# viswavi/speech-anonymization

Hardware: AMD Instinct MI355X
Metric: audio frames/sec (node), ConvAE+gender-adv train step (higher is better)
Workload: dtype bf16x3; 1 GPU; ConvAE recon0.1+sex0.9 adversarial train step (L1 recon + NLL), shape M: 32 utt/GPU x 161120 samples (T=1008 frames), Fbank x2 + norm + fwd + bwd + clip + Adam + Noam; batch_per_gpu=32, frames_per_utt=1008, parallelism=dp1

## Files before the change

include/sa_hip.h:

```cpp
#ifndef SA_HIP_H
#define SA_HIP_H
#ifdef __cplusplus
extern "C" {
#endif

#define SA_F32 0
#define SA_BF16 1
#define SA_BF16X3 2
#define SA_BF16X1F 3
#define SA_FP8 4
#define SA_F64 5
#define SA_MAX_TAPS 5
#define SA_COMM_ID_BYTES 128

typedef struct SaTaps {
  int ntaps[2];
  int off[2][SA_MAX_TAPS];
  int widx[2][SA_MAX_TAPS];
} SaTaps;

typedef struct SaConvArgs {
  const void* x;
  const void* wp;
  const float* bias;
// ... 19 lines not shown
} SaConvArgs;

int sa_conv_gemm(int dtype, int cin, int cout, int sa, int u, const SaConvArgs* a, void* stream);
int sa_abi_sizeof(int which);
int sa_conv_gemm_ntiles(int cin, int cout, int u, int Lout);
int sa_conv_gemm_ntiles_tm(int tile_rows, int u, int Lout);
int sa_conv_gemm_set_tile_rows(int rows);
int sa_conv_gemm_geometry(int dtype, int cin, int cout, int u, int Lout, int* ntiles, int* nslabs);
int sa_conv_gemm_set_impl(int impl);
int sa_conv_gemm_route(int dtype, int cin, int cout, int sa, int u, const SaConvArgs* a);
int sa_conv_pp_set_tile_rows(int rows);
int sa_conv_ws_set_bcost(int tiles);
int sa_conv_ws_set_xcd_weights(const unsigned char* w8);
int sa_conv_ws_calibrate_read(unsigned long long* life512x2);
int sa_conv_wsd_set_bcost(int tiles);

int sa_pack_weights(int dtype, const float* src, void* dst, int ntaps, int K, int N, int sk, int sn,
                    int st, void* stream);

typedef struct SaPackDesc {
  const float* src; void* dst;
  int dtype, ntaps, K, N, sk, sn, st, pad_;
  float* scale;
} SaPackDesc;
int sa_pack_weights_multi(const SaPackDesc* descs, int n, int blocks_per_image, void* stream);
int sa_pack_scales_multi(const SaPackDesc* descs, int n, void* stream);

typedef struct SaWgradArgs {
  const void* x;
  const void* dy;
// ... 187 lines not shown
```

speech-anonymization_amd/_lib.py:

```python
import ctypes as C
import os

import torch

_HERE = os.path.dirname(os.path.abspath(__file__))
LIB_PATH = os.environ.get("SA_HIP_LIB") or os.path.join(_HERE, "libsa_hip.so")

F32, BF16, BF16X3, BF16X1F, FP8, F64 = 0, 1, 2, 3, 4, 5
MAX_TAPS = 5

c_fp = C.POINTER(C.c_float)
vp = C.c_void_p


class SaTaps(C.Structure):
    _fields_ = [("ntaps", C.c_int * 2), ("off", (C.c_int * MAX_TAPS) * 2),
                ("widx", (C.c_int * MAX_TAPS) * 2)]


class SaConvArgs(C.Structure):
    _fields_ = [("x", vp), ("wp", vp), ("bias", vp), ("y", vp),
                ("s1", vp), ("t1", vp), ("s2", vp), ("t2", vp),
                ("swish", C.c_int), ("relu", C.c_int), ("stats", vp),
                ("B", C.c_int), ("Lin", C.c_int), ("Lout", C.c_int), ("ntiles", C.c_int),
# ... 77 lines not shown


SYMBOLS = [
    "sa_conv_gemm", "sa_abi_sizeof", "sa_conv_gemm_ntiles", "sa_conv_gemm_ntiles_tm", "sa_conv_gemm_set_tile_rows",
    "sa_conv_gemm_geometry", "sa_conv_gemm_set_impl", "sa_conv_gemm_route", "sa_conv_pp_set_tile_rows", "sa_pack_weights", "sa_pack_weights_multi", "sa_pack_scales_multi", "sa_wgrad", "sa_wgrad_kw", "sa_wgrad_reduce",
    "sa_conv1toC", "sa_conv1toC_ntiles", "sa_convCto1", "sa_wgrad1C", "sa_wgrad1C_nchunk",
    "sa_sum_slabs", "sa_ew_stats", "sa_ew_apply", "sa_ew_ntiles", "sa_act_stats",
    "sa_sum_partials", "sa_sum_rows_d", "sa_reduce_finalize", "sa_fin_in_fwd", "sa_fin_bn_fwd", "sa_fin_bn_eval", "sa_fin_norm_bwd", "sa_fin_bias",
    "sa_pool_fwd", "sa_pool_nseg", "sa_pool_gather", "sa_pool_fin", "sa_pool_bwd", "sa_dense", "sa_colsums",
    "sa_bn2d_bwd", "sa_dense_wgrad", "sa_log_softmax", "sa_log_softmax_bwd",
    "sa_loss_workspace_bytes", "sa_recon_loss", "sa_cls_losses", "sa_cosine_loss",
    "sa_tdnn_fwd", "sa_time_pool", "sa_leaky_affine", "sa_tdnn_bwd_input", "sa_tdnn_fold", "sa_time_pool_bwd",
    "sa_leaky_affine_bwd", "sa_cluster_mi", "sa_fbank", "sa_fbank_table_elems", "sa_fbank_ntiles", "sa_fbank_scratch_bytes", "sa_fbank_normalize",
    "sa_comm_unique_id", "sa_comm_init", "sa_comm_world", "sa_comm_allreduce", "sa_comm_allreduce_inline", "sa_comm_join", "sa_comm_ncalls",
    "sa_comm_destroy", "sa_head_fwd", "sa_head_bwd", "sa_head_max_rows", "sa_conv_ws_set_bcost", "sa_conv_wsd_set_bcost",
    "sa_add_layernorm_fwd", "sa_layernorm_bwd", "sa_reflect_pad_fwd", "sa_reflect_pad_bwd", "sa_ln_leaky_fwd", "sa_ln_leaky_bwd", "sa_bias_multi", "sa_asr_block0_fwd", "sa_asr_block0_bwd", "sa_conv_ws_set_xcd_weights", "sa_conv_ws_calibrate_read", "sa_wgrad_reduce_multi", "sa_clip_grads",
]

_lib = None


class SaHipError(RuntimeError):
    pass


def load():
    global _lib
    if _lib is None:
        if not os.path.exists(LIB_PATH):
            raise SaHipError(
                f"{LIB_PATH} not found: build it with `python -c 'import __graft_entry__ as g; "
# ... 52 lines not shown
```

speech-anonymization_amd/csrc/sa_conv_ws.hip:

```cpp
#include <type_traits>
#include "sa_conv_cfg.h"

#ifndef SA_ABL
#define SA_ABL 0
#endif

#ifdef SA_WS_STAMPS
__device__ unsigned long long sa_ws_dbg[64 * 8];
#define WS_STAMP(it, i) do { if (lane_ == 0 && wave_ == 0 && blockIdx.x == 7 && (it) < 64) { \
  unsigned long long t_; asm volatile("s_memtime %0\n\ts_waitcnt lgkmcnt(0)" : "=s"(t_) :: "memory"); \
  sa_ws_dbg[(it) * 8 + (i)] = t_; } } while (0)
extern "C" int sa_ws_dbg_read(unsigned long long* out) {
  return -(int)hipMemcpyFromSymbol(out, HIP_SYMBOL(sa_ws_dbg), sizeof(sa_ws_dbg));
}
#else
#define WS_STAMP(it, i)
#endif

#include "sa_conv_ws_common.h"

extern unsigned long long g_ws_xcd_weights;

namespace {

template <int MODE, int NT, int HALO, int CC = 128, int CO = CC, int SA = 1, int UU = 1>
__global__ __launch_bounds__(256) __attribute__((amdgpu_waves_per_eu(1, 1)))
void sa_conv_ws_kernel(SaConvArgs a, int bcost, int total_tiles, unsigned long long xw) {
  typedef WsGeo<CC, NT, HALO, CO, SA, UU> G;
  constexpr int WS_CO = G::CO, WS_SA = G::SA, WS_BM = G::BM;
  static_assert(UU == 1 || MODE == 0, "transposed layers: plain rows");
  constexpr int WS_C = G::C, WS_TM = G::TM, WS_KSTEPS = G::KSTEPS, WS_PITCH = G::PITCH, RPP = G::RPP, LPR = G::LPR,
                NWN = G::NWN, NWM = G::NWM;
  static_assert(CC == 128 || MODE == 0 || MODE == 1, "64 channels: plain and affine + x*sigmoid(x) prologues");
  constexpr int WS_NTAPS = G::NTAPS, WS_ROWS = G::ROWS, WS_PLANE = G::PLANE, WS_NDMA = G::NDMA, WS_DPW = G::DPW,
                WS_RAW_BYTES = G::RAW_BYTES, WS_BUF_BYTES = G::BUF_BYTES, WS_NAGPR_FRAGS = G::NAGPR_FRAGS,
                WS_FT = G::FT, WS_SUBS = G::SUBS;
  (void)WS_ROWS; (void)NWM;
  static_assert(MODE == 0 || MODE == 5 || NT == 5, "the staged transforms need the 240-slot tile");
  constexpr bool PRO2 = MODE == 2;
  constexpr bool SWISH = MODE == 1 || MODE == 3 || MODE == 4;
  constexpr bool PSTAT = MODE == 3, AFF2 = MODE == 4 || MODE == 5;
  constexpr bool COLRED = PRO2 || PSTAT;
  extern __shared__ __attribute__((aligned(16))) unsigned char smem[];
  bf16_t* const planes = reinterpret_cast<bf16_t*>(smem);
  unsigned char* const raw = smem + 2 * WS_BUF_BYTES;
  const unsigned raw_lds = (unsigned)(uintptr_t)(lds_byte*)raw;
  const int tid = threadIdx.x, lane_ = tid & 63;
  const int wave_ = __builtin_amdgcn_readfirstlane(tid >> 6);
  const int wn_ = wave_ % NWN, wm_ = wave_ / NWN;
  const int ph_ = UU == 2 ? wm_ % 2 : 0, rh_ = UU == 2 ? wm_ / 2 : wm_;
  const int ntap_ = a.taps.ntaps[ph_];
#ifdef SA_WS_OLD_RANGES
  int first, last;
  {
    const unsigned long long U = (unsigned long long)a.ntiles + 4u;
    const unsigned long long ctot = (unsigned long long)(total_tiles / a.ntiles) * U;
    auto inv = [&](unsigned long long c) {
// ... 66 lines not shown
  float bv = a.bias ? a.bias[wn_ * 32 + (lane_ & 31)] : 0.0f;
  float relu_floor = a.relu ? 0.0f : -__builtin_inff();
  const bool has_stats = a.stats != nullptr, has_ao = a.a_out != nullptr;

  const int half_ = lane_ >> 5, l31_ = lane_ & 31;
  const int rowp_ = lane_ / LPR, cq_ = lane_ % LPR;
  unsigned row0 = RPP * wave_ + rowp_;
  unsigned dma_off = wave_ * 1024 + lane_ * 16;
  unsigned raw_off = wave_ * 1024 + lane_ * 16;
  unsigned pl_off = (row0 * WS_PITCH + cq_ * 4) * 2;
  unsigned ao_off = (row0 * WS_C + cq_ * 4) * 2;
  unsigned y_off = (UU == 2 ? (8 * half_ + ph_ + 128 * rh_) * WS_CO + wn_ * 32 + l31_
                            : (4 * half_ + 64 * rh_) * WS_CO + wn_ * 32 + l31_) * 4;
  unsigned st_off = ((G::SLABS == 2 ? rh_ * WS_CO : 0) + wn_ * 32 + l31_) * 8;
  unsigned swap_off = (lane_ ^ 32) * 4;
  asm volatile("" : "+v"(bv), "+v"(relu_floor), "+v"(row0), "+v"(dma_off), "+v"(raw_off), "+v"(pl_off), "+v"(ao_off), "+v"(y_off),
               "+v"(st_off), "+v"(swap_off));

#define WS_IDS int lane = lane_, wave = wave_; asm volatile("" : "+v"(lane), "+s"(wave)); (void)wave; (void)lane

  struct Tile { int b, tile, irow, orow, srow; };
  const int slab_short = G::SLABS == 2 ? 2 * a.ntiles - (((a.Lout + UU - 1) / UU + 63) / 64) : 0;
  const int nslab_b = a.ntiles * G::SLABS - slab_short;
  auto tile_of = [&](int t) {
    Tile r; r.b = t / a.ntiles; r.tile = t - r.b * a.ntiles;
    r.irow = r.b * a.Lin + r.tile * (WS_BM * WS_SA) + a.rowmin; r.orow = r.b * a.Lout + r.tile * WS_TM;
    r.srow = r.b * nslab_b + r.tile * G::SLABS;
    return r;
  };
  const int iwrap = a.Lin - (a.ntiles - 1) * (WS_BM * WS_SA), owrap = a.Lout - (a.ntiles - 1) * WS_TM,
            swrap = nslab_b - (a.ntiles - 1) * G::SLABS;
  auto next_tile = [&](Tile T) {
// ... 173 lines not shown
      if (j == WS_DPW - 1 && wave_ + 4 * j >= WS_NDMA) return;
      if (owns(T, false, j)) {
#pragma unroll
        for (int q = 0; q < 4; ++q) { csum[q] += f[q]; csq[q] = fmaf(f[q], f[q], csq[q]); }
      }
    }
  };
  auto piece_write = [&](int j, int part = 2) {
    if (j == WS_DPW - 1 && wave_ + 4 * j >= WS_NDMA) return;
    unsigned char* dst = smem + (pl_cur + j * (4 * RPP * WS_PITCH * 2));
    if (part != 1) *reinterpret_cast<uint2*>(dst) = phi;
    if (part != 0) *reinterpret_cast<uint2*>(dst + WS_PLANE * 2) = plo;
  };
  auto piece_cache = [&](Tile T, bool edge, int j) {
    if (j == WS_DPW - 1 && wave_ + 4 * j >= WS_NDMA) return;
    if (has_ao && owns(T, edge, j)) ws_store_b64(aobase_t + j * (4 * RPP * WS_C * 2), ao_off, phi);
  };
  constexpr int NRED = PSTAT ? 2 : 1;
  auto colsum_put = [&](int it) {
    if constexpr (COLRED) {
      if (PSTAT || a.nb_colsum) {
        float* colred = reinterpret_cast<float*>(raw + (PRO2 ? 2 : 1) * WS_RAW_BYTES) + (size_t)(it & 1) * 4 * WS_C * NRED;
#pragma unroll
        for (int q = 0; q < 4; ++q) {
          const float v = csum[q] + __int_as_float(__builtin_amdgcn_ds_bpermute((int)swap_off, __float_as_int(csum[q])));
          if (lane_ < 32) colred[(wave_ * WS_C + (lane_ & 31) * 4 + q) * NRED] = v;
          csum[q] = 0.0f;
          if constexpr (PSTAT) {
            const float u = csq[q] + __int_as_float(__builtin_amdgcn_ds_bpermute((int)swap_off, __float_as_int(csq[q])));
            if (lane_ < 32) colred[(wave_ * WS_C + (lane_ & 31) * 4 + q) * NRED + 1] = u;
            csq[q] = 0.0f;
          }
        }
      }
    }
  };
  auto colsum_out = [&](int t, int it) {
    if constexpr (COLRED) {
      if ((PSTAT || a.nb_colsum) && tid < WS_C) {
        const float* colred = reinterpret_cast<const float*>(raw + (PRO2 ? 2 : 1) * WS_RAW_BYTES) + (size_t)(it & 1) * 4 * WS_C * NRED;
        float* dst = PSTAT ? a.pro_stats : a.nb_colsum;
// ... 5 lines not shown
      }
    }
  };

  f32x16 acc[2], accp[2];
  float ssum = 0.0f, ssq = 0.0f;
  auto epi_form = [&](int n) {
    float val = accp[n >> 4][n & 15] + bv;
    asm("v_max_f32 %0, %0, %1" : "+v"(val) : "v"(relu_floor));
    return val;
  };
  float eval = 0.0f;
  auto epi_store = [&](int n) {
    const int m = n >> 4, i = n & 15;
    const int ro = m * 32 + (i & 3) + 8 * (i >> 2);
    if constexpr ((SA_ABL & 64) == 0) ws_store_b32(ybase_e + ro * (UU * WS_CO * 4), y_off, eval);
  };
  auto epi_accum = [&](int n) {
    asm volatile("v_add_f32 %0, %0, %2\n\tv_fmac_f32 %1, %2, %2" : "+v"(ssum), "+v"(ssq) : "v"(eval));
    if (n + 1 < 32) eval = epi_form(n + 1);
  };
  auto epi_value = [&](Tile T, bool partial, int n) {
    if (!partial) {
      epi_store(n);
      epi_accum(n);
    } else {
      WS_IDS;
      const int m = n >> 4, i = n & 15;
      const int ro = m * 32 + (i & 3) + 8 * (i >> 2);
      const float val = epi_form(n);
      const int orow = UU == 2 ? 2 * (64 * rh_ + ro + 4 * (lane >> 5)) + ph_ : 64 * rh_ + ro + 4 * (lane >> 5);
// ... 4 lines not shown
    }
  };
  float st_s = 0.0f, st_q = 0.0f;
  bool st_slab_ok = true;
  bool st_pending = false;
  int st_it = 0;
  char* stbase_e = nullptr;
  auto epi_stats = [&](Tile T, int part = 2) {
    if (has_stats) {
      if (part != 1) {
        st_s = ssum + __int_as_float(__builtin_amdgcn_ds_bpermute((int)swap_off, __float_as_int(ssum)));
        st_q = ssq + __int_as_float(__builtin_amdgcn_ds_bpermute((int)swap_off, __float_as_int(ssq)));
      }
      if (part != 0) {
        if constexpr (G::COMBINE == 1) {
          ws_store_b64(stbase_e, st_off, make_uint2(__float_as_uint(st_s), __float_as_uint(st_q)));
        } else {
          float2* stred = reinterpret_cast<float2*>(raw + WS_RAW_BYTES) + (size_t)(st_it & 1) * 4 * 32;
          if (lane_ < 32) stred[wave_ * 32 + lane_] = make_float2(st_s, st_q);
          st_pending = true;
        }
      }
    }
    if (part != 0) { ssum = 0.0f; ssq = 0.0f; }
  };
  auto stats_out = [&]() {
    if constexpr (G::COMBINE == 2) {
      const bool leader = UU == 2 ? ph_ == 0 : wm_ == 0;
      if (st_pending && leader && st_slab_ok) {
        const float2* stred = reinterpret_cast<const float2*>(raw + WS_RAW_BYTES) + (size_t)(st_it & 1) * 4 * 32;
        const float2 p0 = stred[wave_ * 32 + (lane_ & 31)], p1 = stred[(wave_ + NWN) * 32 + (lane_ & 31)];
        ws_store_b64(stbase_e, st_off, make_uint2(__float_as_uint(p0.x + p1.x), __float_as_uint(p0.y + p1.y)));
      }
      st_pending = false;
      ++st_it;
    }
  };

  int toff[WS_NTAPS];
#pragma unroll
  for (int t = 0; t < WS_NTAPS; ++t) toff[t] = (a.taps.off[ph_][UU == 1 || t < ntap_ ? t : 0] - a.rowmin) * WS_PITCH;

  Tile Tc = tile_of(first), Tn = tile_of(first + 1 < last ? first + 1 : last - 1), Tp = Tc;
#pragma unroll
  for (int q = 0; q < 4; ++q) { csum[q] = 0.0f; csq[q] = 0.0f; }
  {
    const bool ec = is_edge(Tc), en = is_edge(Tn);
// ... 58 lines not shown
    }
    WS_STAMP(it, 0);
    auto tile_body = [&](auto fast_c) {
      constexpr bool FAST = decltype(fast_c)::value;
      auto filler = [&](auto f_c) {
        constexpr int fs = decltype(f_c)::value;
        if constexpr ((SA_ABL & 8) != 0 || !FAST) return;
        if constexpr (fs < 32) {
          epi_store(fs); epi_accum(fs);
        } else if constexpr (fs == 32 || fs == 33) {
          epi_stats(Tp, fs - 32);
        } else if constexpr (fs == 34) {
          WS_STAMP(it, 3);
        } else if constexpr (fs == WS_FT - 1) {
          WS_STAMP(it, 4);
          if (G::COMBINE == 1 && has_stats) asm volatile("s_waitcnt vmcnt(33)" ::: "memory");
          else asm volatile("s_waitcnt vmcnt(32)" ::: "memory");
          WS_STAMP(it, 5);
          piece_read(0);
        } else if constexpr (fs >= WS_FT && WS_SUBS == 18) {
          constexpr int j = (fs - WS_FT) / 18, k = (fs - WS_FT) % 18;
          constexpr int NA = AFF2 ? 7 : 6;
          if constexpr (j > 0 && (k == 6 || k == 7)) piece_write(j - 1, k - 6);
          if constexpr (k < NA) piece_level(Tn, j, k);
          if constexpr (j + 1 < WS_DPW && k == 1) piece_read(j + 1, 0);
          if constexpr (j + 1 < WS_DPW && k == 13 && PRO2) piece_read(j + 1, 1);
          if constexpr (k >= 8 && k < 12) piece_split(j, k - 8);
          if constexpr (k == 14) piece_cache(Tn, false, j);
          if constexpr (k == 15) piece_pstat(Tn, j);
          if constexpr (k == 16) dma_piece(Tnn, false, j, 0);
          if constexpr (k == 17 && PRO2) dma_piece(Tnn, false, j, 1);
        } else if constexpr (fs >= WS_FT && WS_SUBS == 4) {
          constexpr int j = (fs - WS_FT) / 4, k = (fs - WS_FT) % 4;
          if constexpr (j > 0 && k < 2) piece_write(j - 1, k);
          if constexpr (k == 0) { piece_level(Tn, j, 0); piece_split(j, 0); }
          if constexpr (j + 1 < WS_DPW && k == 1) piece_read(j + 1, 0);
          if constexpr (k == 1) piece_split(j, 1);
          if constexpr (k == 2) { piece_split(j, 2); piece_split(j, 3); }
          if constexpr (k == 3) { piece_cache(Tn, false, j); dma_piece(Tnn, false, j); }
        } else if constexpr (fs >= WS_FT && WS_SUBS == 6) {
          constexpr int j = (fs - WS_FT) / 6, k = (fs - WS_FT) % 6;
          if constexpr (j > 0 && k < 2) piece_write(j - 1, k);
          if constexpr (k == 0) { piece_level(Tn, j, 0); piece_level(Tn, j, 1); }
          if constexpr (j + 1 < WS_DPW && k == 1) piece_read(j + 1, 0);
          if constexpr (k == 1) { piece_level(Tn, j, 2); piece_level(Tn, j, 3); }
          if constexpr (k == 2) { piece_level(Tn, j, 4); piece_level(Tn, j, 5); }
          if constexpr (k == 3) { piece_split(j, 0); piece_split(j, 1); }
          if constexpr (k == 4) { piece_split(j, 2); piece_split(j, 3); }
          if constexpr (k == 5) { piece_cache(Tn, false, j); dma_piece(Tnn, false, j); }
        } else if constexpr (fs >= WS_FT) {
          constexpr int j = (fs - WS_FT) / 12, k = (fs - WS_FT) % 12;
          if constexpr (j > 0 && k < 2) piece_write(j - 1, k);
          if constexpr (k == 0) piece_level(Tn, j, 0);
          if constexpr (j + 1 < WS_DPW && k == 1) piece_read(j + 1, 0);
// ... 159 lines not shown
}

unsigned long long g_ws_xcd_weights = 0x4040404040404040ull;

extern "C" int sa_conv_ws_set_xcd_weights(const unsigned char* w8) {
  if (!w8) return -22;
  unsigned long long v = 0;
  for (int x = 0; x < 8; ++x) {
    if (w8[x] < 16) return -22;
    v |= (unsigned long long)w8[x] << (8 * x);
  }
  g_ws_xcd_weights = v;
  return 0;
}

extern "C" int sa_conv_ws_set_bcost(int tiles) {
  if ((tiles & 0xffff) < 4 || (tiles & 0xffff) > 64 || (tiles & ~0x1ffff)) return -22;
  g_ws_bcost = tiles;
  return 0;
}

bool sa_conv_ws_covers(int dtype, int cin, int cout, int sa, int u, const SaConvArgs* a) {
  if (dtype == SA_BF16X3 && ((cin == 128 && cout == 64) || (cin == 64 && cout == 32)) && sa == 1 && u == 2) {
    if (a->taps.ntaps[0] > 3 || a->taps.ntaps[1] > 3 || a->taps.ntaps[0] < 1 || a->taps.ntaps[1] < 1) return false;
    int lo = 1 << 30, hi = -(1 << 30);
    for (int ph = 0; ph < 2; ++ph)
      for (int t = 0; t < a->taps.ntaps[ph]; ++t) {
        lo = a->taps.off[ph][t] < lo ? a->taps.off[ph][t] : lo;
        hi = a->taps.off[ph][t] > hi ? a->taps.off[ph][t] : hi;
      }
    if (hi - lo != 2 || lo > 0 || hi < 0) return false;
    if (a->tile_rows && a->tile_rows != 128) return false;
    return !a->s1 && !a->swish && !a->s2 && !a->t2 && !a->pro_stats && !a->nb_x && !a->ep_mode && !a->wscale && !a->relu;
  }
  const bool s2layer = cin == 64 && cout == 128 && sa == 2;
  if (dtype != SA_BF16X3 || u != 1 || !(s2layer || (cin == cout && sa == 1 && (cin == 128 || cin == 64)))) return false;
  const int nt = a->taps.ntaps[0];
  if (cin == 64 && (nt != 5 || a->s2 || a->t2 || a->pro_stats || a->nb_x)) return false;
  if ((nt != 5 && nt != 3) || a->wscale) return false;
  if (a->ep_mode) return false;
  int omin = 1 << 30, omax = -(1 << 30);
  for (int t = 0; t < nt; ++t) {
    omin = a->taps.off[0][t] < omin ? a->taps.off[0][t] : omin;
    omax = a->taps.off[0][t] > omax ? a->taps.off[0][t] : omax;
  }
  if (nt == 5 ? omax - omin != 4 : (omax - omin != 4 && omax - omin != 6)) return false;
  if ((a->a_out || a->nb_colsum || a->pro_stats) && (omin > 0 || (omin & 1))) return false;
  if (a->tile_rows && a->tile_rows != (cout == 64 ? 128 : 64)) return false;
#ifndef SA_WS_PRO2
  if (a->nb_x) return false;
#else
  if (a->nb_x) return nt == 5 && !a->s1 && !a->swish && a->nb_c1 && a->nb_c2 && a->nb_c3;
#endif
  if (nt == 3)
    return !a->s1 && !a->swish && !a->pro_stats && (a->s2 || !a->t2);
  if ((a->s2 || a->t2) && (!a->s2 || !a->s1 || a->pro_stats)) return false;
  if (a->pro_stats && !a->s1) return false;
  if (a->s1) return a->t1 && a->swish;
  return !a->swish;
}

int sa_conv_ws_tile_rows(int cout) { return cout == 128 ? 64 : 128; }
int sa_conv_ws_rows_per_tile(int cout) { return cout == 128 ? 64 : cout == 64 ? 128 : 256; }

int sa_conv_ws_dispatch(int cin, int cout, const SaConvArgs* a, hipStream_t st) {
  if (cin == 128 && cout == 64) return launch_ws<0, 3, 2, 128, 64, 1, 2>(*a, st);
  if (cin == 64 && cout == 32) return launch_ws<0, 3, 2, 64, 32, 1, 2>(*a, st);
  if (cin == 64 && cout == 128) return a->s1 ? launch_ws<1, 5, 4, 64, 128, 2>(*a, st) : launch_ws<0, 5, 4, 64, 128, 2>(*a, st);
  if (cin == 64) return a->s1 ? launch_ws<1, 5, 4, 64>(*a, st) : launch_ws<0, 5, 4, 64>(*a, st);
  if (a->taps.ntaps[0] == 3) {
    int omin = 1 << 30, omax = -(1 << 30);
    for (int t = 0; t < 3; ++t) {
      omin = a->taps.off[0][t] < omin ? a->taps.off[0][t] : omin;
      omax = a->taps.off[0][t] > omax ? a->taps.off[0][t] : omax;
    }
    if (omax - omin == 4) return a->s2 ? launch_ws<5, 3, 4>(*a, st) : launch_ws<0, 3, 4>(*a, st);
    return a->s2 ? launch_ws<5, 3, 6>(*a, st) : launch_ws<0, 3, 6>(*a, st);
  }
#ifdef SA_WS_PRO2
  if (a->nb_x) return launch_ws<2>(*a, st);
#endif
  if (a->s1 && a->pro_stats) return launch_ws<3>(*a, st);
  if (a->s1 && a->s2) return launch_ws<4>(*a, st);
// ... 4 lines not shown
```

speech-anonymization_amd/csrc/sa_conv_ws_common.h:

```cpp
#pragma once
#include <type_traits>
#include "sa_conv_cfg.h"

namespace {

template <int C_, int NT, int HALO_, int CO_ = C_, int SA_ = 1, int U_ = 1>
struct WsGeo {
  static constexpr int C = C_, CO = CO_, SA = SA_, U = U_, NTAPS = NT, HALO = HALO_;
  static constexpr int NWN = CO_ / 32, NWM = 4 / NWN;
  static_assert(U_ == 1 || NWM == 2 || NWM == 4, "two phases = wave pairs of a column block");
  static constexpr int RHW = NWM / U_;
  static constexpr int BM = 64 * RHW;
  static constexpr int SLABS = U_ == 2 ? RHW : 1, COMBINE = NWM / SLABS;
  static constexpr int TM = BM * U_;
  static constexpr int KSTEPS = C_ / 16;
  static constexpr int PITCH = C_ + 8;
  static constexpr int RPP = 256 / C_;
  static constexpr int LPR = 64 / RPP;
  static constexpr int ROWS = ((BM - 1) * SA_ + 1 + HALO_ + RPP - 1) / RPP * RPP;
  static constexpr int PLANE = ROWS * PITCH;
  static constexpr int NDMA = ROWS / RPP;
  static constexpr int DPW = (NDMA + 3) / 4;
  static constexpr int RAW_BYTES = ROWS * C_ * 4;
  static constexpr int BUF_BYTES = 2 * PLANE * 2;
// ... 5 lines not shown
};

typedef __attribute__((address_space(3))) unsigned char lds_byte;

__device__ static inline void ws_dma16(const void* gsrc, unsigned lds_dst) {
  unsigned keep;
  asm volatile("s_mov_b32 %0, m0\n\ts_mov_b32 m0, %2\n\ts_nop 0\n\tglobal_load_lds_dwordx4 %1, off\n\ts_mov_b32 m0, %0"
               : "=&s"(keep) : "v"(gsrc), "s"(lds_dst) : "memory");
}
__device__ static inline void ws_dma16s(const void* gbase, unsigned voff, unsigned lds_dst) {
  unsigned keep;
  asm volatile("s_mov_b32 %0, m0\n\ts_mov_b32 m0, %3\n\ts_nop 0\n\tglobal_load_lds_dwordx4 %1, %2\n\ts_mov_b32 m0, %0"
               : "=&s"(keep) : "v"(voff), "s"(gbase), "s"(lds_dst) : "memory");
}

__device__ static inline void ws_store_b32(void* base, unsigned voff, float v) {
  asm volatile("global_store_dword %0, %1, %2" :: "v"(voff), "v"(v), "s"(base) : "memory");
}
__device__ static inline void ws_store_b64(void* base, unsigned voff, uint2 v) {
  asm volatile("global_store_dwordx2 %0, %1, %2" :: "v"(voff), "v"(v), "s"(base) : "memory");
}

__device__ static inline unsigned ws_cvt_pk_bf16(float a, float b) {
  unsigned r;
  asm("v_cvt_pk_bf16_f32 %0, %1, %2" : "=v"(r) : "v"(a), "v"(b));
  return r;
}

template <int I, int N, class F>
__device__ __forceinline__ void ws_static_for(F&& f) {
  if constexpr (I < N) {
    f(std::integral_constant<int, I>{});
    ws_static_for<I + 1, N>(f);
  }
// ... 4 lines not shown
```

speech-anonymization_amd/csrc/sa_conv_wsd.hip:

```cpp
#include "sa_conv_ws_common.h"

#ifndef SA_WSD_ABL
#define SA_WSD_ABL 0
#endif

#ifdef SA_WSD_STAMPS
__device__ unsigned long long sa_wsd_dbg[64 * 16];
__device__ unsigned long long sa_wsd_wg[512 * 2];
#define WSD_WG_STAMP(i) do { if (lane_ == 0 && wave_ == 0 && blockIdx.x < 512) { \
  unsigned long long t_; asm volatile("s_memrealtime %0\n\ts_waitcnt lgkmcnt(0)" : "=s"(t_) :: "memory"); \
  sa_wsd_wg[blockIdx.x * 2 + (i)] = t_; } } while (0)
#define WSD_STAMP(it, i) do { if (lane_ == 0 && wave_ == 0 && blockIdx.x == 7 && (it) < 64) { \
  unsigned long long t_; asm volatile("s_memtime %0\n\ts_waitcnt lgkmcnt(0)" : "=s"(t_) :: "memory"); \
  sa_wsd_dbg[(it) * 16 + (i)] = t_; } } while (0)
#define WSD_STAMP_RT(it, i) do { if (lane_ == 0 && wave_ == 0 && blockIdx.x == 7 && (it) < 64) { \
  unsigned long long t_; asm volatile("s_memrealtime %0\n\ts_waitcnt lgkmcnt(0)" : "=s"(t_) :: "memory"); \
  sa_wsd_dbg[(it) * 16 + (i)] = t_; } } while (0)
extern "C" int sa_wsd_dbg_read(unsigned long long* out) {
  return -(int)hipMemcpyFromSymbol(out, HIP_SYMBOL(sa_wsd_dbg), sizeof(sa_wsd_dbg));
}
extern "C" int sa_wsd_wg_read(unsigned long long* out) {
  return -(int)hipMemcpyFromSymbol(out, HIP_SYMBOL(sa_wsd_wg), sizeof(sa_wsd_wg));
}
#else
#define WSD_STAMP(it, i)
#define WSD_STAMP_RT(it, i)
#define WSD_WG_STAMP(i)
#endif

extern unsigned long long g_ws_xcd_weights;
__device__ unsigned long long sa_wsd_life[512 * 2];
#define WSD_LIFE(i) do { if (threadIdx.x == 0 && blockIdx.x < 512) { \
  unsigned long long t_; asm volatile("s_memrealtime %0\n\ts_waitcnt lgkmcnt(0)" : "=s"(t_) :: "memory"); \
  sa_wsd_life[blockIdx.x * 2 + (i)] = t_; } } while (0)

namespace {

template <int NT_, int HALO_, int PRO_, int EP_>
struct WsdSched {
  typedef WsGeo<128, NT_, HALO_> G;
  static constexpr int NS = NT_ * G::KSTEPS;
  static constexpr int SECT = NS * 3;
  static constexpr int DPW = G::DPW;
  static constexpr int NP0 = (DPW + 1) / 2, NP1 = DPW - NP0;
  static constexpr int LPV = EP_ == 4 ? 2 : 1;
  static constexpr int EII = EP_ == 1 || EP_ == 4 ? 3 : EP_ == 3 ? 2 : 1;
  static constexpr int ELV = EP_ == 1 ? 11 : EP_ == 4 ? 13 : EP_ == 3 ? 9 : 3;
// ... 316 lines not shown
    }
    if (lv == 2) {
#pragma unroll
      for (int q = 0; q < 4; ++q) w[q] = f[q] - z[q];
    }
    if (lv == 3) { plo.x = ws_cvt_pk_bf16(w[0], w[1]); plo.y = ws_cvt_pk_bf16(w[2], w[3]); }
  };
  auto piece_write = [&](int j, int part = 2) {
    if (!has_piece(j)) return;
    unsigned char* dst = smem + (pl_cur + j * (4 * RPP * WS_PITCH * 2));
    if (part != 1) *reinterpret_cast<uint2*>(dst) = phi;
    if (part != 0) *reinterpret_cast<uint2*>(dst + WS_PLANE * 2) = plo;
  };
  auto piece_cache = [&](Tile T, bool edge, int j) {
    if (!has_piece(j)) return;
    if (has_ao && owns(T, edge, j)) ws_store_b64(aobase_t + j * (4 * RPP * WS_C * 2), ao_off, phi);
  };
  auto colsum_put = [&](int it) {
    if constexpr (PRO2) {
      if (a.nb_colsum) {
        float* colred = reinterpret_cast<float*>(raw + 2 * WS_RAW_BYTES) + (size_t)(it & 1) * 4 * WS_C;
        f32x4 v;
#pragma unroll
        for (int q = 0; q < 4; ++q) {
          const auto r = __builtin_amdgcn_permlane32_swap(__float_as_uint(csum[q]), __float_as_uint(csum[q]), false, false);
          v[q] = __uint_as_float(r[0]) + __uint_as_float(r[1]);
        }
        if (lane_ < 32) *reinterpret_cast<f32x4*>(colred + wave_ * WS_C + (lane_ & 31) * 4) = v;
      }
#pragma unroll
      for (int q = 0; q < 4; ++q) csum[q] = 0.0f;
// ... 108 lines not shown
      (void)&ssum; (void)&ssq; (void)&y_off;
      if (in_bounds(i)) {
        ws_static_for<0, Sch::ELV>([&](auto lv_c) { epi_level(h_c, i_c, lv_c); });
        epi_store(i_c, yb + WSD_Q(h, i) * (16 * WS_C * 4));
      }
    });
  };
  char* stbase_p = nullptr;
  auto epi_stats = [&]() {
    if (has_stats) {
      const auto rs = __builtin_amdgcn_permlane32_swap(__float_as_uint(ssum), __float_as_uint(ssum), false, false);
      const auto rq = __builtin_amdgcn_permlane32_swap(__float_as_uint(ssq), __float_as_uint(ssq), false, false);
      const float st_s = __uint_as_float(rs[0]) + __uint_as_float(rs[1]);
      const float st_q = __uint_as_float(rq[0]) + __uint_as_float(rq[1]);
      WS_IDS;
      ws_store_b64(stbase_p, (unsigned)((wave * 32 + (lane & 31)) * 8), make_uint2(__float_as_uint(st_s), __float_as_uint(st_q)));
    }
    ssum = 0.0f; ssq = 0.0f;
  };
  auto drain_vmem = [&]() {
    asm volatile("s_waitcnt vmcnt(0)" ::: "memory");
  };

  int toff[WS_NTAPS];
#pragma unroll
  for (int t = 0; t < WS_NTAPS; ++t) toff[t] = (a.taps.off[0][t] - a.rowmin) * WS_PITCH;

  Tile Tc = tile_of(first), Tn = tile_of(first + 1 < last ? first + 1 : last - 1), Tp = Tc;
#pragma unroll
  for (int q = 0; q < 4; ++q) csum[q] = 0.0f;
  {
// ... 264 lines not shown
  SaConvArgs args = a;
  args.ntiles = sa_div_up(a.Lout, G::BM);
  int omin = 1 << 30, omax = -(1 << 30), wmax = 0;
  for (int t = 0; t < NT; ++t) {
    omin = a.taps.off[0][t] < omin ? a.taps.off[0][t] : omin;
    omax = a.taps.off[0][t] > omax ? a.taps.off[0][t] : omax;
    wmax = a.taps.widx[0][t] > wmax ? a.taps.widx[0][t] : wmax;
  }
  if (omax - omin != HALO) return -22;
  args.rowmin = omin;
  args.nrows = G::ROWS;
  args.wlo_off = (wmax + 1) * G::KSTEPS * 4 * 64;
  if ((a.a_out || a.nb_colsum) && (omin > 0 || omax < 0 || (args.ntiles - 1) * G::BM + omin + G::ROWS < a.Lin))
    return -22;
  if ((long)a.B * a.Lin >= (1L << 31) - 64 || (long)a.B * a.Lout >= (1L << 31) - 64) return -22;
  const size_t lds = 2 * G::BUF_BYTES + (PRO == 2 ? 2 : 1) * G::RAW_BYTES + (PRO == 2 ? 2 * 4 * 128 * 4 : 0);
  if (lds > 160 * 1024) return -12;
  auto kern = sa_conv_wsd_kernel<NT, HALO, PRO, EP>;
  static bool attr_set = false;
  static int n_cu = 0;
  if (!attr_set) {
    hipError_t e = hipFuncSetAttribute(reinterpret_cast<const void*>(kern),
                                       hipFuncAttributeMaxDynamicSharedMemorySize, 160 * 1024);
    if (e != hipSuccess) return -(int)e;
    int dev = 0;
    hipDeviceProp_t prop;
    if (hipGetDevice(&dev) != hipSuccess || hipGetDeviceProperties(&prop, dev) != hipSuccess) return -19;
    n_cu = prop.multiProcessorCount;
    attr_set = true;
  }
  const int total = args.ntiles * a.B;
  const int nwg = total < n_cu ? total : n_cu;
// ... 6 lines not shown
  if (dtype != SA_BF16X3 || cin != 128 || cout != 128 || sa != 1 || u != 1) return 0;
  if (a->ep_mode != 1 && a->ep_mode != 2) return 0;
  if (!a->ep_x || !a->ep_mean || !a->ep_rstd || !a->stats) return 0;
  if (a->s1 || a->t1 || a->s2 || a->t2 || a->swish || a->relu || a->pro_stats || a->wscale || a->bias) return 0;
  if (a->tile_rows && a->tile_rows != 64) return 0;
  const int nt = a->taps.ntaps[0];
  if (nt != 5 && nt != 3) return 0;
  int omin = 1 << 30, omax = -(1 << 30);
  for (int t = 0; t < nt; ++t) {
    omin = a->taps.off[0][t] < omin ? a->taps.off[0][t] : omin;
    omax = a->taps.off[0][t] > omax ? a->taps.off[0][t] : omax;
  }
  const int halo = omax - omin;
  if (nt == 5 ? halo != 4 : (halo != 4 && halo != 6)) return 0;
  if (omin > 0 || (omin & 1) || omax < 0) return 0;
  int pro, ep;
  if (a->nb_x) {
    if (!a->nb_c1 || !a->nb_c2 || !a->nb_c3) return 0;
    pro = 2;
  } else {
    if (a->a_out || a->nb_colsum) return 0;
    pro = 0;
  }
  if (a->ep_mode == 1) {
    if (!a->ep_s1 || !a->ep_t1 || a->ep_xp_is_act || a->ep_bstride != 128) return 0;
    if (a->ep_g2) { if (!a->ep_g2k1 || !a->ep_g2k2 || !a->ep_g2k3) return 0; ep = 4; } else ep = 1;
  } else {
    if (a->ep_g2 || a->ep_bstride != 0) return 0;
    if (a->ep_xp_is_act) { if (!a->ep_s1 || !a->ep_t1) return 0; ep = 3; } else { if (a->ep_s1 || a->ep_t1) return 0; ep = 2; }
  }
  if (pro == 2 && (a->nb_relu_mask != 0) != (ep != 1)) return 0;
  if (nt == 5 && pro == 2 && ep == 1) return 1;
  if (nt == 5 && pro == 2 && ep == 3) return 2;
  if (nt == 5 && pro == 0 && ep == 4) return 3;
  if (nt == 3 && halo == 4 && pro == 2 && ep == 2) return 4;
  if (nt == 3 && halo == 6 && pro == 2 && ep == 2) return 5;
  return 0;
}

}

extern "C" int sa_conv_wsd_set_bcost(int tiles) {
  if ((tiles & 0xffff) < 4 || (tiles & 0xffff) > 64 || (tiles & ~0x1ffff)) return -22;
  g_wsd_bcost = tiles;
  return 0;
}

extern "C" int sa_conv_ws_calibrate_read(unsigned long long* life512x2) {
  if (!life512x2) return -22;
  return -(int)hipMemcpyFromSymbol(life512x2, HIP_SYMBOL(sa_wsd_life), sizeof(sa_wsd_life));
}

bool sa_conv_wsd_covers(int dtype, int cin, int cout, int sa, int u, const SaConvArgs* a) {
  return wsd_variant(dtype, cin, cout, sa, u, a) != 0;
}

int sa_conv_wsd_dispatch(int cin, int cout, const SaConvArgs* a, hipStream_t st) {
  switch (wsd_variant(SA_BF16X3, cin, cout, 1, 1, a)) {
// ... 9 lines not shown
```

speech-anonymization_amd/ops.py:

```python
import ctypes as C
import functools

import torch

from . import _lib as L

UP2 = [[(1, 0), (0, 2), (-1, 4)], [(1, 1), (0, 3)]]


def taps_conv(K, dil, pad):
    return [[(k * dil - pad, k) for k in range(K)]]


def taps_conv_dgrad_s1(K, dil, pad):
    return [[(pad - k * dil, k) for k in range(K)]]


def taps_convT_dgrad(K=5, pad=2):
    return [[(k - pad, k) for k in range(K)]]


def _f(t):
    return L.ptr(t)

# ... 176 lines not shown
        kind = (f"sa_conv_wsd_kernel ({tname}, {cin}->{cout}; 5 instances)" if route == 3 else
                f"sa_conv_ws_kernel<{ws_mode},{ntap}> ({tname}, {cin}->{cout})" if route == 2 else
                f"sa_conv_pp_kernel<{tname},{cin},{cout},{sa},{u}>" if route == 1 else
                f"sa_conv_gemm_kernel<{tname},{cin},{cout},{sa},{u}{',nb prologue' if nb else ''}>")
        PROFILE.stop(e0, io + ntap * cin * cout * esz + extra,
                     2 * B * (-(-Lout // u)) * ntap * cin * cout,
                     alg_bytes=io + (y.numel() * esz if ep else 0), kind=kind)
    out_t = (y, stats) if want_stats else (y,)
    if nb and nb.get("want_colsum"):
        out_t = out_t + (colsum,)
    if want_pro_stats:
        out_t = out_t + (pro_stats,)
    return out_t if len(out_t) > 1 else y


if __import__("os").environ.get("SA_WS_FIRST_PLAIN") == "1":
    L.load().sa_conv_ws_set_bcost(9 | 0x10000)
    L.load().sa_conv_wsd_set_bcost(9 | 0x10000)

WGRAD_TARGET_WGS = {True: 256, False: 512}
if __import__("os").environ.get("SA_WG_TARGETS"):
    _b, _s = __import__("os").environ["SA_WG_TARGETS"].split(",")
    WGRAD_TARGET_WGS = {True: int(_b), False: int(_s)}


def wgrad(x, dy, cin, cout, sa, u, taps, Mrows, dst, dst_strides, s1=None, t1=None, s2=None,
          t2=None, swish=False, accumulate=False, target_wgs=None, code=None, x_pre=False,
          dy_pre=False, defer=None):
    lib = L.load()
    B, Lin, _ = x.shape
    Ldy = dy.shape[1]
    if x_pre:
        assert x.dtype == torch.bfloat16 and code in (L.BF16X1F, L.BF16)
# ... 468 lines not shown
    w = (torch.randn(128, 128, 5, generator=g) * 0.05).to(dev)
    wd = pack_weights(w, "conv_dgrad", torch.float32, L.BF16X3)
    c = [(torch.rand(B, 128, generator=g) + 0.5).to(dev) for _ in range(3)]
    s1 = (torch.rand(B, 128, generator=g) + 0.5).to(dev)
    ao = torch.empty(B, Lin, 128, device=dev, dtype=torch.bfloat16)
    out = torch.empty(B, Lin, 128, device=dev)
    kw = dict(code=L.BF16X3, want_stats=True, a_out=ao, out=out,
              nb=dict(x=y2, c1=c[0], c2=c[1], c3=c[2], per_c=False, relu_mask=False, want_colsum=True),
              ep=dict(mode=1, x=xe, s1=s1, t1=s1, mean=s1, rstd=s1))
    weights = [64] * 8
    buf = (C.c_ulonglong * 1024)()
    for r in range(rounds + 1):
        L.check(lib.sa_conv_ws_set_xcd_weights((C.c_ubyte * 8)(*weights)), "sa_conv_ws_set_xcd_weights")
        if r == rounds:
            break
        for _ in range(3):
            conv_gemm(x, wd, None, 128, 128, 1, 1, taps_conv_dgrad_s1(5, 1, 2), Lin, **kw)
        torch.cuda.synchronize(dev)
        L.check(lib.sa_conv_ws_calibrate_read(buf), "sa_conv_ws_calibrate_read")
        life = [[] for _ in range(8)]
        for i in range(512):
            if buf[2 * i] and buf[2 * i + 1] > buf[2 * i]:
                life[i % 8].append(buf[2 * i + 1] - buf[2 * i])
        if any(len(v) < 4 for v in life):
            break
        med = [sorted(v)[len(v) // 2] for v in life]
        speed = [weights[xi] / med[xi] for xi in range(8)]
        mean = sum(speed) / 8.0
        weights = [max(32, min(128, int(round(64.0 * sp / mean)))) for sp in speed]
        if verbose:
            print(f"[calibrate_xcd] round {r}: median lifetime by XCD (us) {[round(m * 0.01, 1) for m in med]} -> weights {weights}",
                  flush=True)
# ... 16 lines not shown
```

Baseline: 3.830 million frames/s.

## Route stride-2 64->128 normalisation-backward conv through the warp-specialised kernel

Adds a MODE 2 (normalisation-backward prologue) instantiation of the warp-specialised conv kernel for the stride-2 64->128 layer. It adds a 16-lane column-sum reduction path and a PRO2 sub-step schedule, and routes calls with nb_x to it by default, with an SA_WS_SMALL=0 switch to turn it off. It also gates the wsd lifetime timestamp writes behind a calibration bit so normal runs skip them. The cost is extra kernel specialisation and a full vmcnt wait in the PRO2 path.

```diff
diff --git a/include/sa_hip.h b/include/sa_hip.h
--- a/include/sa_hip.h
+++ b/include/sa_hip.h
@@ -57,6 +57,7 @@
 int sa_conv_ws_set_xcd_weights(const unsigned char* w8);
 int sa_conv_ws_calibrate_read(unsigned long long* life512x2);
 int sa_conv_wsd_set_bcost(int tiles);
+int sa_conv_ws_set_small(int on);
 
 int sa_pack_weights(int dtype, const float* src, void* dst, int ntaps, int K, int N, int sk, int sn,
                     int st, void* stream);
diff --git a/speech-anonymization_amd/_lib.py b/speech-anonymization_amd/_lib.py
--- a/speech-anonymization_amd/_lib.py
+++ b/speech-anonymization_amd/_lib.py
@@ -115,7 +115,7 @@
     "sa_leaky_affine_bwd", "sa_cluster_mi", "sa_fbank", "sa_fbank_table_elems", "sa_fbank_ntiles", "sa_fbank_scratch_bytes", "sa_fbank_normalize",
     "sa_comm_unique_id", "sa_comm_init", "sa_comm_world", "sa_comm_allreduce", "sa_comm_allreduce_inline", "sa_comm_join", "sa_comm_ncalls",
     "sa_comm_destroy", "sa_head_fwd", "sa_head_bwd", "sa_head_max_rows", "sa_conv_ws_set_bcost", "sa_conv_wsd_set_bcost",
-    "sa_add_layernorm_fwd", "sa_layernorm_bwd", "sa_reflect_pad_fwd", "sa_reflect_pad_bwd", "sa_ln_leaky_fwd", "sa_ln_leaky_bwd", "sa_bias_multi", "sa_asr_block0_fwd", "sa_asr_block0_bwd", "sa_conv_ws_set_xcd_weights", "sa_conv_ws_calibrate_read", "sa_wgrad_reduce_multi", "sa_clip_grads",
+    "sa_add_layernorm_fwd", "sa_layernorm_bwd", "sa_reflect_pad_fwd", "sa_reflect_pad_bwd", "sa_ln_leaky_fwd", "sa_ln_leaky_bwd", "sa_bias_multi", "sa_asr_block0_fwd", "sa_asr_block0_bwd", "sa_conv_ws_set_xcd_weights", "sa_conv_ws_calibrate_read", "sa_conv_ws_set_small", "sa_wgrad_reduce_multi", "sa_clip_grads",
 ]
 
 _lib = None
diff --git a/speech-anonymization_amd/csrc/sa_conv_ws.hip b/speech-anonymization_amd/csrc/sa_conv_ws.hip
--- a/speech-anonymization_amd/csrc/sa_conv_ws.hip
+++ b/speech-anonymization_amd/csrc/sa_conv_ws.hip
@@ -31,7 +31,8 @@
   static_assert(UU == 1 || MODE == 0, "transposed layers: plain rows");
   constexpr int WS_C = G::C, WS_TM = G::TM, WS_KSTEPS = G::KSTEPS, WS_PITCH = G::PITCH, RPP = G::RPP, LPR = G::LPR,
                 NWN = G::NWN, NWM = G::NWM;
-  static_assert(CC == 128 || MODE == 0 || MODE == 1, "64 channels: plain and affine + x*sigmoid(x) prologues");
+  static_assert(CC == 128 || MODE == 0 || MODE == 1 || (MODE == 2 && SA == 2 && CO == 128),
+                "64 channels: plain and affine + x*sigmoid(x) prologues; the stride-2 layer also the normalisation-backward one");
   constexpr int WS_NTAPS = G::NTAPS, WS_ROWS = G::ROWS, WS_PLANE = G::PLANE, WS_NDMA = G::NDMA, WS_DPW = G::DPW,
                 WS_RAW_BYTES = G::RAW_BYTES, WS_BUF_BYTES = G::BUF_BYTES, WS_NAGPR_FRAGS = G::NAGPR_FRAGS,
                 WS_FT = G::FT, WS_SUBS = G::SUBS;
@@ -41,6 +42,7 @@
   constexpr bool SWISH = MODE == 1 || MODE == 3 || MODE == 4;
   constexpr bool PSTAT = MODE == 3, AFF2 = MODE == 4 || MODE == 5;
   constexpr bool COLRED = PRO2 || PSTAT;
+  static_assert(!PRO2 || G::COMBINE == 1, "the statistics scratch of two row halves overlays the raw nb_x tile");
   extern __shared__ __attribute__((aligned(16))) unsigned char smem[];
   bf16_t* const planes = reinterpret_cast<bf16_t*>(smem);
   unsigned char* const raw = smem + 2 * WS_BUF_BYTES;
@@ -137,8 +139,9 @@
                             : (4 * half_ + 64 * rh_) * WS_CO + wn_ * 32 + l31_) * 4;
   unsigned st_off = ((G::SLABS == 2 ? rh_ * WS_CO : 0) + wn_ * 32 + l31_) * 8;
   unsigned swap_off = (lane_ ^ 32) * 4;
+  unsigned swap16_off = (lane_ ^ 16) * 4;
   asm volatile("" : "+v"(bv), "+v"(relu_floor), "+v"(row0), "+v"(dma_off), "+v"(raw_off), "+v"(pl_off), "+v"(ao_off), "+v"(y_off),
-               "+v"(st_off), "+v"(swap_off));
+               "+v"(st_off), "+v"(swap_off), "+v"(swap16_off));
 
 #define WS_IDS int lane = lane_, wave = wave_; asm volatile("" : "+v"(lane), "+s"(wave)); (void)wave; (void)lane
 
@@ -342,7 +345,7 @@
   };
   auto piece_cache = [&](Tile T, bool edge, int j) {
     if (j == WS_DPW - 1 && wave_ + 4 * j >= WS_NDMA) return;
-    if (has_ao && owns(T, edge, j)) ws_store_b64(aobase_t + j * (4 * RPP * WS_C * 2), ao_off, phi);
+    if (has_ao && owns(T, edge, j)) ws_gstore_b64(aobase_t + j * (4 * RPP * WS_C * 2), ao_off, phi);
   };
   constexpr int NRED = PSTAT ? 2 : 1;
   auto colsum_put = [&](int it) {
@@ -351,8 +354,10 @@
         float* colred = reinterpret_cast<float*>(raw + (PRO2 ? 2 : 1) * WS_RAW_BYTES) + (size_t)(it & 1) * 4 * WS_C * NRED;
 #pragma unroll
         for (int q = 0; q < 4; ++q) {
-          const float v = csum[q] + __int_as_float(__builtin_amdgcn_ds_bpermute((int)swap_off, __float_as_int(csum[q])));
-          if (lane_ < 32) colred[(wave_ * WS_C + (lane_ & 31) * 4 + q) * NRED] = v;
+          float v = csum[q];
+          if constexpr (LPR == 16) v += __int_as_float(__builtin_amdgcn_ds_bpermute((int)swap16_off, __float_as_int(v)));
+          v += __int_as_float(__builtin_amdgcn_ds_bpermute((int)swap_off, __float_as_int(v)));
+          if (lane_ < LPR) colred[(wave_ * WS_C + (lane_ % LPR) * 4 + q) * NRED] = v;
           csum[q] = 0.0f;
           if constexpr (PSTAT) {
             const float u = csq[q] + __int_as_float(__builtin_amdgcn_ds_bpermute((int)swap_off, __float_as_int(csq[q])));
@@ -388,7 +393,7 @@
   auto epi_store = [&](int n) {
     const int m = n >> 4, i = n & 15;
     const int ro = m * 32 + (i & 3) + 8 * (i >> 2);
-    if constexpr ((SA_ABL & 64) == 0) ws_store_b32(ybase_e + ro * (UU * WS_CO * 4), y_off, eval);
+    if constexpr ((SA_ABL & 64) == 0) ws_gstore_b32(ybase_e + ro * (UU * WS_CO * 4), y_off, eval);
   };
   auto epi_accum = [&](int n) {
     asm volatile("v_add_f32 %0, %0, %2\n\tv_fmac_f32 %1, %2, %2" : "+v"(ssum), "+v"(ssq) : "v"(eval));
@@ -423,7 +428,7 @@
       }
       if (part != 0) {
         if constexpr (G::COMBINE == 1) {
-          ws_store_b64(stbase_e, st_off, make_uint2(__float_as_uint(st_s), __float_as_uint(st_q)));
+          ws_gstore_b64(stbase_e, st_off, make_uint2(__float_as_uint(st_s), __float_as_uint(st_q)));
         } else {
           float2* stred = reinterpret_cast<float2*>(raw + WS_RAW_BYTES) + (size_t)(st_it & 1) * 4 * 32;
           if (lane_ < 32) stred[wave_ * 32 + lane_] = make_float2(st_s, st_q);
@@ -439,7 +444,7 @@
       if (st_pending && leader && st_slab_ok) {
         const float2* stred = reinterpret_cast<const float2*>(raw + WS_RAW_BYTES) + (size_t)(st_it & 1) * 4 * 32;
         const float2 p0 = stred[wave_ * 32 + (lane_ & 31)], p1 = stred[(wave_ + NWN) * 32 + (lane_ & 31)];
-        ws_store_b64(stbase_e, st_off, make_uint2(__float_as_uint(p0.x + p1.x), __float_as_uint(p0.y + p1.y)));
+        ws_gstore_b64(stbase_e, st_off, make_uint2(__float_as_uint(p0.x + p1.x), __float_as_uint(p0.y + p1.y)));
       }
       st_pending = false;
       ++st_it;
@@ -528,7 +533,8 @@
           WS_STAMP(it, 3);
         } else if constexpr (fs == WS_FT - 1) {
           WS_STAMP(it, 4);
-          if (G::COMBINE == 1 && has_stats) asm volatile("s_waitcnt vmcnt(33)" ::: "memory");
+          if (PRO2) asm volatile("s_waitcnt vmcnt(0)" ::: "memory");
+          else if (G::COMBINE == 1 && has_stats) asm volatile("s_waitcnt vmcnt(33)" ::: "memory");
           else asm volatile("s_waitcnt vmcnt(32)" ::: "memory");
           WS_STAMP(it, 5);
           piece_read(0);
@@ -552,6 +558,16 @@
           if constexpr (k == 1) piece_split(j, 1);
           if constexpr (k == 2) { piece_split(j, 2); piece_split(j, 3); }
           if constexpr (k == 3) { piece_cache(Tn, false, j); dma_piece(Tnn, false, j); }
+        } else if constexpr (fs >= WS_FT && WS_SUBS == 6 && PRO2) {
+          constexpr int j = (fs - WS_FT) / 6, k = (fs - WS_FT) % 6;
+          if constexpr (j > 0 && k < 2) piece_write(j - 1, k);
+          if constexpr (k == 0) { piece_level(Tn, j, 0); piece_level(Tn, j, 1); }
+          if constexpr (k == 1) piece_level(Tn, j, 2);
+          if constexpr (j + 1 < WS_DPW && k == 1) piece_read(j + 1);
+          if constexpr (k == 2) { piece_level(Tn, j, 3); piece_split(j, 0); }
+          if constexpr (k == 3) { piece_split(j, 1); piece_split(j, 2); }
+          if constexpr (k == 4) piece_split(j, 3);
+          if constexpr (k == 5) { piece_cache(Tn, false, j); dma_piece(Tnn, false, j); }
         } else if constexpr (fs >= WS_FT && WS_SUBS == 6) {
           constexpr int j = (fs - WS_FT) / 6, k = (fs - WS_FT) % 6;
           if constexpr (j > 0 && k < 2) piece_write(j - 1, k);
@@ -741,6 +757,13 @@
   return 0;
 }
 
+static bool g_ws_small = true;
+extern "C" int sa_conv_ws_set_small(int on) {
+  if (on != 0 && on != 1) return -22;
+  g_ws_small = on != 0;
+  return 0;
+}
+
 extern "C" int sa_conv_ws_set_bcost(int tiles) {
   if ((tiles & 0xffff) < 4 || (tiles & 0xffff) > 64 || (tiles & ~0x1ffff)) return -22;
   g_ws_bcost = tiles;
@@ -762,8 +785,9 @@
   }
   const bool s2layer = cin == 64 && cout == 128 && sa == 2;
   if (dtype != SA_BF16X3 || u != 1 || !(s2layer || (cin == cout && sa == 1 && (cin == 128 || cin == 64)))) return false;
+  if ((long)a->B * a->Lin >= (1L << 31) - 64 || (long)a->B * a->Lout >= (1L << 31) - 64) return false;
   const int nt = a->taps.ntaps[0];
-  if (cin == 64 && (nt != 5 || a->s2 || a->t2 || a->pro_stats || a->nb_x)) return false;
+  if (cin == 64 && (nt != 5 || a->s2 || a->t2 || a->pro_stats || (a->nb_x && !s2layer))) return false;
   if ((nt != 5 && nt != 3) || a->wscale) return false;
   if (a->ep_mode) return false;
   int omin = 1 << 30, omax = -(1 << 30);
@@ -774,6 +798,14 @@
   if (nt == 5 ? omax - omin != 4 : (omax - omin != 4 && omax - omin != 6)) return false;
   if ((a->a_out || a->nb_colsum || a->pro_stats) && (omin > 0 || (omin & 1))) return false;
   if (a->tile_rows && a->tile_rows != (cout == 64 ? 128 : 64)) return false;
+  if (s2layer && a->nb_x) {
+    typedef WsGeo<64, 5, 4, 128, 2> G;
+    int omin = 1 << 30;
+    for (int t = 0; t < nt; ++t) omin = a->taps.off[0][t] < omin ? a->taps.off[0][t] : omin;
+    const int ntiles = sa_div_up(a->Lout, G::BM);
+    if ((a->a_out || a->nb_colsum) && (long)(ntiles - 1) * G::BM * 2 + omin + G::ROWS < a->Lin) return false;
+    return g_ws_small && !a->s1 && !a->swish && a->nb_c1 && a->nb_c2 && a->nb_c3;
+  }
 #ifndef SA_WS_PRO2
   if (a->nb_x) return false;
 #else
@@ -793,7 +825,9 @@
 int sa_conv_ws_dispatch(int cin, int cout, const SaConvArgs* a, hipStream_t st) {
   if (cin == 128 && cout == 64) return launch_ws<0, 3, 2, 128, 64, 1, 2>(*a, st);
   if (cin == 64 && cout == 32) return launch_ws<0, 3, 2, 64, 32, 1, 2>(*a, st);
-  if (cin == 64 && cout == 128) return a->s1 ? launch_ws<1, 5, 4, 64, 128, 2>(*a, st) : launch_ws<0, 5, 4, 64, 128, 2>(*a, st);
+  if (cin == 64 && cout == 128)
+    return a->nb_x ? launch_ws<2, 5, 4, 64, 128, 2>(*a, st)
+           : a->s1 ? launch_ws<1, 5, 4, 64, 128, 2>(*a, st) : launch_ws<0, 5, 4, 64, 128, 2>(*a, st);
   if (cin == 64) return a->s1 ? launch_ws<1, 5, 4, 64>(*a, st) : launch_ws<0, 5, 4, 64>(*a, st);
   if (a->taps.ntaps[0] == 3) {
     int omin = 1 << 30, omax = -(1 << 30);
diff --git a/speech-anonymization_amd/csrc/sa_conv_ws_common.h b/speech-anonymization_amd/csrc/sa_conv_ws_common.h
--- a/speech-anonymization_amd/csrc/sa_conv_ws_common.h
+++ b/speech-anonymization_amd/csrc/sa_conv_ws_common.h
@@ -43,10 +43,10 @@
                : "=&s"(keep) : "v"(voff), "s"(gbase), "s"(lds_dst) : "memory");
 }
 
-__device__ static inline void ws_store_b32(void* base, unsigned voff, float v) {
+__device__ static inline void ws_gstore_b32(void* base, unsigned voff, float v) {
   asm volatile("global_store_dword %0, %1, %2" :: "v"(voff), "v"(v), "s"(base) : "memory");
 }
-__device__ static inline void ws_store_b64(void* base, unsigned voff, uint2 v) {
+__device__ static inline void ws_gstore_b64(void* base, unsigned voff, uint2 v) {
   asm volatile("global_store_dwordx2 %0, %1, %2" :: "v"(voff), "v"(v), "s"(base) : "memory");
 }
 
diff --git a/speech-anonymization_amd/csrc/sa_conv_wsd.hip b/speech-anonymization_amd/csrc/sa_conv_wsd.hip
--- a/speech-anonymization_amd/csrc/sa_conv_wsd.hip
+++ b/speech-anonymization_amd/csrc/sa_conv_wsd.hip
@@ -30,7 +30,7 @@
 
 extern unsigned long long g_ws_xcd_weights;
 __device__ unsigned long long sa_wsd_life[512 * 2];
-#define WSD_LIFE(i) do { if (threadIdx.x == 0 && blockIdx.x < 512) { \
+#define WSD_LIFE(i) do { if ((bcost & 0x20000) && threadIdx.x == 0 && blockIdx.x < 512) { \
   unsigned long long t_; asm volatile("s_memrealtime %0\n\ts_waitcnt lgkmcnt(0)" : "=s"(t_) :: "memory"); \
   sa_wsd_life[blockIdx.x * 2 + (i)] = t_; } } while (0)
 
@@ -377,7 +377,7 @@
   };
   auto piece_cache = [&](Tile T, bool edge, int j) {
     if (!has_piece(j)) return;
-    if (has_ao && owns(T, edge, j)) ws_store_b64(aobase_t + j * (4 * RPP * WS_C * 2), ao_off, phi);
+    if (has_ao && owns(T, edge, j)) ws_gstore_b64(aobase_t + j * (4 * RPP * WS_C * 2), ao_off, phi);
   };
   auto colsum_put = [&](int it) {
     if constexpr (PRO2) {
@@ -516,7 +516,7 @@
       const float st_s = __uint_as_float(rs[0]) + __uint_as_float(rs[1]);
       const float st_q = __uint_as_float(rq[0]) + __uint_as_float(rq[1]);
       WS_IDS;
-      ws_store_b64(stbase_p, (unsigned)((wave * 32 + (lane & 31)) * 8), make_uint2(__float_as_uint(st_s), __float_as_uint(st_q)));
+      ws_gstore_b64(stbase_p, (unsigned)((wave * 32 + (lane & 31)) * 8), make_uint2(__float_as_uint(st_s), __float_as_uint(st_q)));
     }
     ssum = 0.0f; ssq = 0.0f;
   };
@@ -811,8 +811,8 @@
   if ((a.a_out || a.nb_colsum) && (omin > 0 || omax < 0 || (args.ntiles - 1) * G::BM + omin + G::ROWS < a.Lin))
     return -22;
   if ((long)a.B * a.Lin >= (1L << 31) - 64 || (long)a.B * a.Lout >= (1L << 31) - 64) return -22;
-  const size_t lds = 2 * G::BUF_BYTES + (PRO == 2 ? 2 : 1) * G::RAW_BYTES + (PRO == 2 ? 2 * 4 * 128 * 4 : 0);
-  if (lds > 160 * 1024) return -12;
+  constexpr size_t lds = 2 * G::BUF_BYTES + (PRO == 2 ? 2 : 1) * G::RAW_BYTES + (PRO == 2 ? 2 * 4 * 128 * 4 : 0);
+  static_assert(lds <= 160 * 1024, "LDS");
   auto kern = sa_conv_wsd_kernel<NT, HALO, PRO, EP>;
   static bool attr_set = false;
   static int n_cu = 0;
@@ -849,6 +849,9 @@
   const int halo = omax - omin;
   if (nt == 5 ? halo != 4 : (halo != 4 && halo != 6)) return 0;
   if (omin > 0 || (omin & 1) || omax < 0) return 0;
+  if ((long)a->B * a->Lin >= (1L << 31) - 64 || (long)a->B * a->Lout >= (1L << 31) - 64) return 0;
+  const int rows = nt == 5 ? WsGeo<128, 5, 4>::ROWS : halo == 4 ? WsGeo<128, 3, 4>::ROWS : WsGeo<128, 3, 6>::ROWS;
+  if ((a->a_out || a->nb_colsum) && (long)(sa_div_up(a->Lout, 64) - 1) * 64 + omin + rows < a->Lin) return 0;
   int pro, ep;
   if (a->nb_x) {
     if (!a->nb_c1 || !a->nb_c2 || !a->nb_c3) return 0;
@@ -876,7 +879,7 @@
 }
 
 extern "C" int sa_conv_wsd_set_bcost(int tiles) {
-  if ((tiles & 0xffff) < 4 || (tiles & 0xffff) > 64 || (tiles & ~0x1ffff)) return -22;
+  if ((tiles & 0xffff) < 4 || (tiles & 0xffff) > 64 || (tiles & ~0x3ffff)) return -22;
   g_wsd_bcost = tiles;
   return 0;
 }
diff --git a/speech-anonymization_amd/ops.py b/speech-anonymization_amd/ops.py
--- a/speech-anonymization_amd/ops.py
+++ b/speech-anonymization_amd/ops.py
@@ -214,9 +214,13 @@
     return out_t if len(out_t) > 1 else y
 
 
+_WSD_BCOST = 9
 if __import__("os").environ.get("SA_WS_FIRST_PLAIN") == "1":
+    _WSD_BCOST = 9 | 0x10000
     L.load().sa_conv_ws_set_bcost(9 | 0x10000)
-    L.load().sa_conv_wsd_set_bcost(9 | 0x10000)
+    L.load().sa_conv_wsd_set_bcost(_WSD_BCOST)
+if __import__("os").environ.get("SA_WS_SMALL") == "0":
+    L.check(L.load().sa_conv_ws_set_small(0), "sa_conv_ws_set_small")
 
 WGRAD_TARGET_WGS = {True: 256, False: 512}
 if __import__("os").environ.get("SA_WG_TARGETS"):
@@ -715,8 +719,12 @@
         L.check(lib.sa_conv_ws_set_xcd_weights((C.c_ubyte * 8)(*weights)), "sa_conv_ws_set_xcd_weights")
         if r == rounds:
             break
-        for _ in range(3):
-            conv_gemm(x, wd, None, 128, 128, 1, 1, taps_conv_dgrad_s1(5, 1, 2), Lin, **kw)
+        L.check(lib.sa_conv_wsd_set_bcost(_WSD_BCOST | 0x20000), "sa_conv_wsd_set_bcost")
+        try:
+            for _ in range(3):
+                conv_gemm(x, wd, None, 128, 128, 1, 1, taps_conv_dgrad_s1(5, 1, 2), Lin, **kw)
+        finally:
+            L.check(lib.sa_conv_wsd_set_bcost(_WSD_BCOST), "sa_conv_wsd_set_bcost")
         torch.cuda.synchronize(dev)
         L.check(lib.sa_conv_ws_calibrate_read(buf), "sa_conv_ws_calibrate_read")
         life = [[] for _ in range(8)]
```

Result: no change. 3.847 million frames/s, median of 6 (+0.4%).
